# parsakhaz/multimodal-image-similarity-search

Hardware: AMD Instinct MI355X
Metric: images/s CLIP-B/32 encode @ bs256; Mvec/s cosine top-10 over 10M x 512 (higher is better)
Workload: dtype bf16

## Files before the change

### multimodal-image-similarity-search_amd/csrc/attention_common.h

```cpp
#pragma once
#include "common.h"
#include "gemm_fp8.h"

#define ATT_VSTRIDE 144

__device__ __forceinline__ float att_max_over_lane_groups(float v) {
    uint32_t u = __float_as_uint(v);
    auto r32 = __builtin_amdgcn_permlane32_swap(u, u, false, false);
    v = mm_max2(__uint_as_float(r32[0]), __uint_as_float(r32[1]));
    u = __float_as_uint(v);
    auto r16 = __builtin_amdgcn_permlane16_swap(u, u, false, false);
    return mm_max2(__uint_as_float(r16[0]), __uint_as_float(r16[1]));
}

struct AttKV { u32x4 k, v; };
__device__ __forceinline__ AttKV att_load_kv_piece(const uint16_t* base, int ld, int dmodel, int row, int c, int T) {
    AttKV t = {u32x4{0u, 0u, 0u, 0u}, u32x4{0u, 0u, 0u, 0u}};
    if (row < T) {
        t.k = *reinterpret_cast<const u32x4*>(base + (size_t)row * ld + dmodel + c * 8);
        t.v = *reinterpret_cast<const u32x4*>(base + (size_t)row * ld + 2 * dmodel + c * 8);
    }
    return t;
}
__device__ __forceinline__ void att_store_kv_piece(char* sK, char* sV, int row, int c, const u32x4 kv, const u32x4 vv) {
    *reinterpret_cast<u32x4*>(sK + row * 128 + ((c ^ (row & 7)) << 4)) = kv;
    *reinterpret_cast<u32x4*>(sV + row * ATT_VSTRIDE + (c << 4)) = vv;
}
template <int ROWS, int NTHR>
__device__ __forceinline__ void att_stage_kv(const uint16_t* base, int ld, int dmodel, int T, int tid, char* sK) {
    for (int idx = tid; idx < ROWS * 8; idx += NTHR) {
        const int row = idx >> 3, c = idx & 7;
        const AttKV t = att_load_kv_piece(base, ld, dmodel, row, c, T);
        att_store_kv_piece(sK, sK + ROWS * 128, row, c, t.k, t.v);
    }
}

__device__ __forceinline__ bf16x8 att_load_q(const uint16_t* base, int ld, int q, int T, int s, int fg) {
    u32x4 raw = {0u, 0u, 0u, 0u};
    if (q < T) raw = *reinterpret_cast<const u32x4*>(base + (size_t)q * ld + s * 32 + fg * 8);
    return __builtin_bit_cast(bf16x8, raw);
}

__device__ __forceinline__ void att_pv_block(const char* vks, const bf16x8& pf, f32x4 (&oacc)[4]) {
#pragma unroll
    for (int dt = 0; dt < 4; ++dt) {
        const char* a0 = vks + dt * 32;
        const bf16x4 v0 = __builtin_amdgcn_ds_read_tr16_b64_v4bf16(
            (__attribute__((address_space(3))) bf16x4*)(a0));
        const bf16x4 v1 = __builtin_amdgcn_ds_read_tr16_b64_v4bf16(
            (__attribute__((address_space(3))) bf16x4*)(a0 + 16 * ATT_VSTRIDE));
        bf16x8 vf;
        vf[0] = v0[0]; vf[1] = v0[1]; vf[2] = v0[2]; vf[3] = v0[3];
        vf[4] = v1[0]; vf[5] = v1[1]; vf[6] = v1[2]; vf[7] = v1[3];
        oacc[dt] = __builtin_amdgcn_mfma_f32_16x16x32_bf16(vf, pf, oacc[dt], 0, 0, 0);
    }
}

#define ATT_C_EXP (0.125f * 1.4426950408889634f)
#define ATT_THR_RAW (8.0f / ATT_C_EXP)

template <bool PAIR, class ScoreTile>
__device__ __forceinline__ void att_key_pair_step(ScoreTile&& score_tile, int ks, const char* vks, const bf16x8& ones, float& m,
                                                  f32x4& lacc, f32x4 (&oacc)[4]) {
    const float c_exp = ATT_C_EXP, thr_raw = ATT_THR_RAW;
    f32x4 p0 = score_tile(2 * ks), p1;
    if constexpr (PAIR) p1 = score_tile(2 * ks + 1);
    else p1 = f32x4{-INFINITY, -INFINITY, -INFINITY, -INFINITY};
    if constexpr (PAIR) mm_mfma_settle("+v"(p0), "+v"(p1));
    else mm_mfma_settle("+v"(p0));
    float lm = mm_max3(p0[0], p0[1], p0[2]);
    if constexpr (PAIR) lm = mm_max3(mm_max3(lm, p0[3], p1[0]), p1[1], mm_max2(p1[2], p1[3]));
    else lm = mm_max2(lm, p0[3]);
    lm = att_max_over_lane_groups(lm);
    if (__any(lm > m + thr_raw)) {
        const float mn = (lm > m + thr_raw) ? lm : m;
        const float alpha = __builtin_amdgcn_exp2f((m - mn) * c_exp);
        m = mn;
#pragma unroll
        for (int dt = 0; dt < 4; ++dt)
#pragma unroll
            for (int r = 0; r < 4; ++r) oacc[dt][r] *= alpha;
#pragma unroll
        for (int r = 0; r < 4; ++r) lacc[r] *= alpha;
    }
    const float mc = m * c_exp;
#pragma unroll
    for (int r = 0; r < 4; ++r) p0[r] = __builtin_amdgcn_exp2f(__builtin_fmaf(p0[r], c_exp, -mc));
#pragma unroll
    for (int r = 0; r < 4; ++r) p1[r] = __builtin_amdgcn_exp2f(__builtin_fmaf(p1[r], c_exp, -mc));
    u32x4 praw;
    praw[0] = pack_bf16x2(p0[0], p0[1]);
    praw[1] = pack_bf16x2(p0[2], p0[3]);
    praw[2] = pack_bf16x2(p1[0], p1[1]);
    praw[3] = pack_bf16x2(p1[2], p1[3]);
    const bf16x8 pf = __builtin_bit_cast(bf16x8, praw);
    lacc = __builtin_amdgcn_mfma_f32_16x16x32_bf16(ones, pf, lacc, 0, 0, 0);
    att_pv_block(vks, pf, oacc);
}

__device__ __forceinline__ void att_store_bf16_row(const f32x4 (&oacc)[4], float inv, uint16_t* orow) {
#pragma unroll
    for (int dt = 0; dt < 4; ++dt) {
        u32x2 pk;
        pk[0] = pack_bf16x2(oacc[dt][0] * inv, oacc[dt][1] * inv);
        pk[1] = pack_bf16x2(oacc[dt][2] * inv, oacc[dt][3] * inv);
        *reinterpret_cast<u32x2*>(orow + dt * 16) = pk;
    }
}

__device__ __forceinline__ void att_store_mx_row(const f32x4 (&oacc)[4], float inv, bool valid, uint8_t* o8row, uint8_t* srow,
                                                 int h, int fg) {
#pragma unroll
    for (int blk = 0; blk < 2; ++blk) {
        float o[2][4];
        float amax = 0.f;
#pragma unroll
        for (int i = 0; i < 2; ++i)
#pragma unroll
            for (int r = 0; r < 4; ++r) {
                o[i][r] = oacc[2 * blk + i][r] * inv;
                amax = fmaxf(amax, fabsf(o[i][r]));
            }
        amax = att_max_over_lane_groups(amax);
        int e8;
        float sinv;
        mx_scale_of(amax, e8, sinv);
        if (valid) {
#pragma unroll
            for (int i = 0; i < 2; ++i)
                *reinterpret_cast<uint32_t*>(o8row + (2 * blk + i) * 16) = pack_fp8x4(o[i][0] * sinv, o[i][1] * sinv, o[i][2] * sinv, o[i][3] * sinv);
            if (fg == 0) srow[mx_scale_offset(2 * h + blk)] = (uint8_t)e8;
        }
    }
}
```

### multimodal-image-similarity-search_amd/csrc/attention_kernels.h

```cpp
#pragma once
#include "attention_common.h"
#include "attention_stream.h"


template <int NKP, bool CAUSAL, bool MXOUT = false>
__device__ __forceinline__ void attention_onepass_tile(const char* sK, const char* sV, const bf16x8 (&qf)[2], int q, int T,
                                                       int fr, int fg, uint16_t* orow, uint8_t* o8row = nullptr, uint8_t* srow = nullptr,
                                                       int h = 0, int only_q = -1) {
    f32x4 sacc[2 * NKP];
    float mx = -INFINITY;
#pragma unroll
    for (int kt = 0; kt < 2 * NKP; ++kt) {
        f32x4 a = {0.f, 0.f, 0.f, 0.f};
        const int krow = kt * 16 + fr;
#pragma unroll
        for (int s = 0; s < 2; ++s) {
            const int chunk = 4 * s + fg;
            const bf16x8 kf = *reinterpret_cast<const bf16x8*>(sK + krow * 128 + ((chunk ^ (krow & 7)) << 4));
            a = __builtin_amdgcn_mfma_f32_16x16x32_bf16(kf, qf[s], a, 0, 0, 0);
        }
#pragma unroll
        for (int r = 0; r < 4; ++r) {
            const int key = kt * 16 + 4 * fg + r;
            const bool ok = (key < T) && (!CAUSAL || key <= q);
            a[r] = ok ? a[r] * 0.125f : -INFINITY;
            mx = fmaxf(mx, a[r]);
        }
        sacc[kt] = a;
    }
    mx = fmaxf(mx, __shfl_xor(mx, 16));
    mx = fmaxf(mx, __shfl_xor(mx, 32));
    float l = 0.f;
#pragma unroll
    for (int kt = 0; kt < 2 * NKP; ++kt)
#pragma unroll
        for (int r = 0; r < 4; ++r) {
            const float pexp = __expf(sacc[kt][r] - mx);
            sacc[kt][r] = pexp;
            l += pexp;
        }
    l += __shfl_xor(l, 16);
    l += __shfl_xor(l, 32);

    f32x4 oacc[4];
#pragma unroll
    for (int dt = 0; dt < 4; ++dt) oacc[dt] = f32x4{0.f, 0.f, 0.f, 0.f};
    const int tq = fr >> 2, tp = fr & 3;
#pragma unroll
    for (int ks = 0; ks < NKP; ++ks) {
        u32x4 praw;
        praw[0] = pack_bf16x2(sacc[2 * ks][0], sacc[2 * ks][1]);
        praw[1] = pack_bf16x2(sacc[2 * ks][2], sacc[2 * ks][3]);
        praw[2] = pack_bf16x2(sacc[2 * ks + 1][0], sacc[2 * ks + 1][1]);
        praw[3] = pack_bf16x2(sacc[2 * ks + 1][2], sacc[2 * ks + 1][3]);
        const bf16x8 pf = __builtin_bit_cast(bf16x8, praw);
#pragma unroll
        for (int dt = 0; dt < 4; ++dt) {
            const char* a0 = sV + (32 * ks + 4 * fg + tq) * ATT_VSTRIDE + (dt * 16 + 4 * tp) * 2;
            const bf16x4 v0 = __builtin_amdgcn_ds_read_tr16_b64_v4bf16(
                (__attribute__((address_space(3))) bf16x4*)(a0));
            const bf16x4 v1 = __builtin_amdgcn_ds_read_tr16_b64_v4bf16(
                (__attribute__((address_space(3))) bf16x4*)(a0 + 16 * ATT_VSTRIDE));
            bf16x8 vf;
            vf[0] = v0[0]; vf[1] = v0[1]; vf[2] = v0[2]; vf[3] = v0[3];
            vf[4] = v1[0]; vf[5] = v1[1]; vf[6] = v1[2]; vf[7] = v1[3];
            oacc[dt] = __builtin_amdgcn_mfma_f32_16x16x32_bf16(vf, pf, oacc[dt], 0, 0, 0);
        }
    }
    const float inv = 1.0f / l;
    if constexpr (MXOUT) {
#pragma unroll
        for (int blk = 0; blk < 2; ++blk) {
            float o[2][4];
            float amax = 0.f;
#pragma unroll
            for (int i = 0; i < 2; ++i)
#pragma unroll
                for (int r = 0; r < 4; ++r) {
                    o[i][r] = oacc[2 * blk + i][r] * inv;
                    amax = fmaxf(amax, fabsf(o[i][r]));
                }
            amax = att_max_over_lane_groups(amax);
            int e8;
            float sinv;
            mx_scale_of(amax, e8, sinv);
            if (q < T) {
#pragma unroll
                for (int i = 0; i < 2; ++i)
                    *reinterpret_cast<uint32_t*>(o8row + (2 * blk + i) * 16) = pack_fp8x4(o[i][0] * sinv, o[i][1] * sinv, o[i][2] * sinv, o[i][3] * sinv);
                if (fg == 0) srow[mx_scale_offset(2 * h + blk)] = (uint8_t)e8;
            }
        }
    } else if (q < T && (only_q < 0 || q == only_q)) {
        att_store_bf16_row(oacc, inv, orow);
    }
}

template <int NKP, bool CAUSAL, bool MXOUT = false>
__global__ __launch_bounds__(256) void attention_kernel(const uint16_t* __restrict__ qkv, uint16_t* __restrict__ ctx, int T, int H,
                                                        uint8_t* __restrict__ ctx8 = nullptr, uint8_t* __restrict__ ctxs = nullptr, int ld_s = 0) {
    static_assert(NKP <= 4, "sequences over 128 keys: attention_long_kernel");
    extern __shared__ __attribute__((aligned(16))) char smem[];
    constexpr int TP = NKP * 32;
    char* sK = smem;
    char* sV = smem + TP * 128;
    const int tid = threadIdx.x, lane = tid & 63, wave = tid >> 6;
    const int b = blockIdx.x / H, h = blockIdx.x - b * H;
    const int dmodel = H * 64, ld = 3 * dmodel;
    const uint16_t* base = qkv + (size_t)b * T * ld + h * 64;

    constexpr int NW = 4;
    const int fr = lane & 15, fg = lane >> 4;
    const int qt_first = wave + NW * blockIdx.y;
    bf16x8 qf_first[2];
#pragma unroll
    for (int s = 0; s < 2; ++s) qf_first[s] = att_load_q(base, ld, qt_first * 16 + fr, T, s, fg);
    att_stage_kv<TP, NW * 64>(base, ld, dmodel, T, tid, sK);
    __syncthreads();

    const int nqt = (T + 15) >> 4;
    for (int qt = qt_first; qt < nqt; qt += NW * gridDim.y) {
        const int q = qt * 16 + fr;
        bf16x8 qf[2];
        if (qt == qt_first) {
            qf[0] = qf_first[0];
            qf[1] = qf_first[1];
        } else {
#pragma unroll
            for (int s = 0; s < 2; ++s) qf[s] = att_load_q(base, ld, q, T, s, fg);
        }
        if constexpr (MXOUT) {
            const size_t row = (size_t)b * T + (q < T ? q : 0);
            attention_onepass_tile<NKP, CAUSAL, true>(sK, sV, qf, q, T, fr, fg, nullptr, ctx8 + row * dmodel + h * 64 + 4 * fg, ctxs + row * ld_s, h);
        } else {
            attention_onepass_tile<NKP, CAUSAL>(sK, sV, qf, q, T, fr, fg, ctx + ((size_t)b * T + q) * dmodel + h * 64 + 4 * fg);
        }
    }
}

template <int NKP, bool CAUSAL, bool MXOUT>
__global__ __launch_bounds__(512) void attention_long_kernel(const uint16_t* __restrict__ qkv, uint16_t* __restrict__ ctx, int T,
                                                             int H, uint8_t* __restrict__ ctx8, uint8_t* __restrict__ ctxs, int ld_s) {
    static_assert(NKP > 4 && NKP <= 9, "129..288 keys");
    extern __shared__ __attribute__((aligned(16))) char smem[];
    constexpr int TP = NKP * 32;
    constexpr int NW = 8;
    char* sK = smem;
    char* sV = smem + TP * 128;
    const int tid = threadIdx.x, lane = tid & 63, wave = tid >> 6;
    const int dmodel = H * 64, ld = 3 * dmodel;
    const int fr = lane & 15, fg = lane >> 4;
    const int nqt = (T + 15) >> 4;
    const char* kbase0 = sK + fr * 128 + ((fg ^ (fr & 7)) << 4);
    const char* kbase1 = sK + fr * 128 + (((4 + fg) ^ (fr & 7)) << 4);
    const int tq = fr >> 2, tp = fr & 3;
    const char* vbase = sV + (4 * fg + tq) * ATT_VSTRIDE + 8 * tp;
    u32x4 ones_raw = {0x3F803F80u, 0x3F803F80u, 0x3F803F80u, 0x3F803F80u};
    asm volatile("" : "+v"(ones_raw));
    const bf16x8 ones = __builtin_bit_cast(bf16x8, ones_raw);

    const int b = blockIdx.x / H, h = blockIdx.x - b * H;
    const uint16_t* base = qkv + (size_t)b * T * ld + h * 64;
    att_stage_kv<TP, NW * 64>(base, ld, dmodel, T, tid, sK);
    __syncthreads();
    for (int qt = wave + NW * blockIdx.y; qt < nqt; qt += NW * gridDim.y) {
        const int q = qt * 16 + fr;
        bf16x8 qf[2];
#pragma unroll
        for (int s = 0; s < 2; ++s) qf[s] = att_load_q(base, ld, q, T, s, fg);
        const int kt_end = CAUSAL ? (qt + 1 < nqt ? qt + 1 : nqt) : nqt;
        const int kt_clean = CAUSAL ? (qt < (T >> 4) ? qt : (T >> 4)) : (T >> 4);
        auto score_tile = [&](int kt) -> f32x4 {
            f32x4 a = {0.f, 0.f, 0.f, 0.f};
            const bf16x8 kf0 = *reinterpret_cast<const bf16x8*>(kbase0 + kt * 2048);
            const bf16x8 kf1 = *reinterpret_cast<const bf16x8*>(kbase1 + kt * 2048);
            a = __builtin_amdgcn_mfma_f32_16x16x32_bf16(kf0, qf[0], a, 0, 0, 0);
            a = __builtin_amdgcn_mfma_f32_16x16x32_bf16(kf1, qf[1], a, 0, 0, 0);
            if (kt >= kt_clean) {
#pragma unroll
                for (int r = 0; r < 4; ++r) {
                    const int key = kt * 16 + 4 * fg + r;
                    const bool ok = (key < T) && (!CAUSAL || key <= q);
                    a[r] = ok ? a[r] : -INFINITY;
                }
            }
            return a;
        };
        float m = -INFINITY;
        f32x4 lacc = {0.f, 0.f, 0.f, 0.f};
        f32x4 oacc[4];
#pragma unroll
        for (int dt = 0; dt < 4; ++dt) oacc[dt] = f32x4{0.f, 0.f, 0.f, 0.f};
        const int npairs = kt_end >> 1;
#pragma unroll 1
        for (int ks = 0; ks < npairs; ++ks) att_key_pair_step<true>(score_tile, ks, vbase + ks * (32 * ATT_VSTRIDE), ones, m, lacc, oacc);
        if (kt_end & 1) att_key_pair_step<false>(score_tile, npairs, vbase + npairs * (32 * ATT_VSTRIDE), ones, m, lacc, oacc);
        const float inv = 1.0f / lacc[0];
        if constexpr (MXOUT) {
            const size_t row = (size_t)b * T + (q < T ? q : 0);
            att_store_mx_row(oacc, inv, q < T, ctx8 + row * dmodel + h * 64 + 4 * fg, ctxs + row * ld_s, h, fg);
        } else if (q < T) {
            att_store_bf16_row(oacc, inv, ctx + ((size_t)b * T + q) * dmodel + h * 64 + 4 * fg);
        }
    }
}

template <int NKP, bool CAUSAL, int HPB, bool MXOUT = false, bool POOLED = false>
__global__ __launch_bounds__(256) void attention_heads_kernel(const uint16_t* __restrict__ qkv, uint16_t* __restrict__ ctx,
                                                              int T, int H, uint8_t* __restrict__ ctx8 = nullptr,
                                                              uint8_t* __restrict__ ctxs = nullptr, int ld_s = 0,
                                                              const int32_t* __restrict__ pool_row = nullptr) {
    static_assert(!(POOLED && MXOUT), "the pooled-query form writes bf16");
    extern __shared__ __attribute__((aligned(16))) char smem[];
    constexpr int TP = NKP * 32;
    constexpr int IMG = TP * (128 + ATT_VSTRIDE);
    const int tid = threadIdx.x, lane = tid & 63, wave = tid >> 6;
    const int fr = lane & 15, fg = lane >> 4;
    const int groups = H / HPB;
    const int b = blockIdx.x / groups, h0 = (blockIdx.x - b * groups) * HPB;
    const int dmodel = H * 64, ld = 3 * dmodel;
    const uint16_t* item = qkv + (size_t)b * T * ld;
    const int nqt = (T + 15) >> 4;

    constexpr int NIT = TP * 8 / 256;
    u32x4 kr[NIT], vr[NIT];
    auto load_head = [&](int h) {
        const uint16_t* base = item + h * 64;
#pragma unroll
        for (int i = 0; i < NIT; ++i) {
            const int idx = tid + i * 256, row = idx >> 3, c = idx & 7;
            kr[i] = u32x4{0u, 0u, 0u, 0u};
            vr[i] = u32x4{0u, 0u, 0u, 0u};
            if (row < T) {
                kr[i] = *reinterpret_cast<const u32x4*>(base + (size_t)row * ld + dmodel + c * 8);
                vr[i] = *reinterpret_cast<const u32x4*>(base + (size_t)row * ld + 2 * dmodel + c * 8);
            }
        }
    };
    auto store_head = [&](int buf) {
        char* sK = smem + buf * IMG;
        char* sV = sK + TP * 128;
#pragma unroll
        for (int i = 0; i < NIT; ++i) {
            const int idx = tid + i * 256, row = idx >> 3, c = idx & 7;
            *reinterpret_cast<u32x4*>(sK + row * 128 + ((c ^ (row & 7)) << 4)) = kr[i];
            *reinterpret_cast<u32x4*>(sV + row * ATT_VSTRIDE + (c << 4)) = vr[i];
        }
    };
    auto load_q = [&](int h, int qt, bf16x8 (&qf)[2]) {
        const int q = qt * 16 + fr;
#pragma unroll
        for (int s = 0; s < 2; ++s) {
            u32x4 raw = {0u, 0u, 0u, 0u};
            if (q < T) raw = *reinterpret_cast<const u32x4*>(item + h * 64 + (size_t)q * ld + s * 32 + fg * 8);
            qf[s] = __builtin_bit_cast(bf16x8, raw);
        }
    };

    bf16x8 qf[2], qn[2];
    int pq = 0, pqt = wave;
    if constexpr (POOLED) {
        pq = __builtin_amdgcn_readfirstlane(pool_row[b]) - b * T;
        pq = pq < 0 ? 0 : (pq >= T ? T - 1 : pq);
        pqt = pq >> 4;
    }
    const bool my_tile = !POOLED || wave == (pqt & 3);
    if constexpr (POOLED) { if (my_tile) load_q(h0, pqt, qf); }
    else load_q(h0, wave, qf);
    load_head(h0);
    store_head(0);
    __syncthreads();
#pragma unroll 1
    for (int hh = 0; hh < HPB; ++hh) {
        const int h = h0 + hh, cur = hh & 1;
        if (hh + 1 < HPB) {
            if constexpr (POOLED) { if (my_tile) load_q(h + 1, pqt, qn); }
            else load_q(h + 1, wave, qn);
            load_head(h + 1);
        }
        const char* sK = smem + cur * IMG;
        const char* sV = sK + TP * 128;
        if constexpr (POOLED) {
            if (my_tile)
                attention_onepass_tile<NKP, CAUSAL>(sK, sV, qf, pqt * 16 + fr, T, fr, fg, ctx + (size_t)b * dmodel + h * 64 + 4 * fg,
                                                    nullptr, nullptr, 0, pq);
        } else
        for (int qt = wave; qt < nqt; qt += 4) {
            const int q = qt * 16 + fr;
            if (qt != wave) load_q(h, qt, qf);
            if constexpr (MXOUT) {
                const size_t row = (size_t)b * T + (q < T ? q : 0);
                attention_onepass_tile<NKP, CAUSAL, true>(sK, sV, qf, q, T, fr, fg, nullptr, ctx8 + row * dmodel + h * 64 + 4 * fg, ctxs + row * ld_s, h);
            } else
            attention_onepass_tile<NKP, CAUSAL>(sK, sV, qf, q, T, fr, fg, ctx + ((size_t)b * T + q) * dmodel + h * 64 + 4 * fg);
        }
        if (hh + 1 < HPB) {
            store_head(cur ^ 1);
            qf[0] = qn[0];
            qf[1] = qn[1];
        }
        __syncthreads();
    }
}

#include "attention_tiled.h"

template <bool MAY_CAUSAL, class F>
static int attention_with_causal(bool causal, F&& f) {
    if constexpr (MAY_CAUSAL)
        if (causal) return f(std::true_type{});
    return f(std::false_type{});
}
template <int LO, int HI, bool MAY_CAUSAL, class F>
static int attention_with_nkp(int T, bool causal, F&& f) {
    if constexpr (LO < HI)
        if ((T + 31) / 32 > LO) return attention_with_nkp<LO + 1, HI, MAY_CAUSAL>(T, causal, f);
    return attention_with_causal<MAY_CAUSAL>(causal, [&](auto causal_tag) -> int { return f(std::integral_constant<int, LO>{}, causal_tag); });
}
template <class F>
static int attention_with_hpb(int hpb, F&& f) {
    switch (hpb) {
        case 2: return f(std::integral_constant<int, 2>{});
        case 3: return f(std::integral_constant<int, 3>{});
        case 4: return f(std::integral_constant<int, 4>{});
        default: return f(std::integral_constant<int, 6>{});
    }
}

static int attention_query_splits(int items, int T, int waves) {
    const int rounds = ((T + 15) / 16 + waves - 1) / waves;
    const int qs = 256 / items;
    return qs < 1 ? 1 : (qs > rounds ? rounds : qs);
}

static int attention_pick_hpb(int B, int H) {
    int hpb = mmiss_option("att_hpb", 0);
    if (hpb == 0) {
        hpb = 1;
        for (int c : {4, 6, 3, 2})
            if (H % c == 0 && (int64_t)B * (H / c) >= 512) { hpb = c; break; }
    }
    return ((hpb == 2 || hpb == 3 || hpb == 4 || hpb == 6) && H % hpb == 0) ? hpb : 1;
}

template <bool MXOUT>
static int launch_attention_short(hipStream_t st, const void* qkv, void* ctx, uint8_t* ctx8, uint8_t* ctxs, int ld_s, int B, int T,
                                  int H, bool causal) {
    const int hpb = attention_pick_hpb(B, H);
    return attention_with_nkp<1, 4, !MXOUT>(T, causal, [&](auto nkp_tag, auto causal_tag) -> int {
        constexpr int NKP = decltype(nkp_tag)::value;
        constexpr bool CAUSAL = decltype(causal_tag)::value;
        constexpr int lds = NKP * 32 * (128 + ATT_VSTRIDE);
        if (hpb > 1)
            return attention_with_hpb(hpb, [&](auto hpb_tag) -> int {
                constexpr int HPB = decltype(hpb_tag)::value;
                MM_TRY(mmiss_ensure_dyn_lds(reinterpret_cast<const void*>(&attention_heads_kernel<NKP, CAUSAL, HPB, MXOUT>), 2 * lds));
                hipLaunchKernelGGL((attention_heads_kernel<NKP, CAUSAL, HPB, MXOUT>), dim3(B * (H / HPB)), dim3(256), 2 * lds, st,
                                   (const uint16_t*)qkv, (uint16_t*)ctx, T, H, ctx8, ctxs, ld_s);
                MM_HIP(hipGetLastError());
                return MMISS_OK;
            });
        MM_TRY(mmiss_ensure_dyn_lds(reinterpret_cast<const void*>(&attention_kernel<NKP, CAUSAL, MXOUT>), lds));
        hipLaunchKernelGGL((attention_kernel<NKP, CAUSAL, MXOUT>), dim3(B * H, attention_query_splits(B * H, T, 4)), dim3(256), lds, st,
                           (const uint16_t*)qkv, (uint16_t*)ctx, T, H, ctx8, ctxs, ld_s);
        MM_HIP(hipGetLastError());
        return MMISS_OK;
    });
}

template <bool MXOUT>
static int launch_attention_long(hipStream_t st, const void* qkv, void* ctx, uint8_t* ctx8, uint8_t* ctxs, int ld_s, int B, int T, int H,
                                 bool causal) {
    if (!causal)
        if (attention_stream_ok(B, T, H, false) && mmiss_option("attention_stream", 1))
            return launch_attention_stream<MXOUT>(st, qkv, ctx, ctx8, ctxs, ld_s, B, H);
    return attention_with_nkp<5, 9, !MXOUT>(T, causal, [&](auto nkp_tag, auto causal_tag) -> int {
        constexpr int NKP = decltype(nkp_tag)::value;
        constexpr bool CAUSAL = decltype(causal_tag)::value;
        constexpr int lds = NKP * 32 * (128 + ATT_VSTRIDE);
        MM_TRY(mmiss_ensure_dyn_lds(reinterpret_cast<const void*>(&attention_long_kernel<NKP, CAUSAL, MXOUT>), lds));
        hipLaunchKernelGGL((attention_long_kernel<NKP, CAUSAL, MXOUT>), dim3(B * H, attention_query_splits(B * H, T, 8)), dim3(512), lds,
                           st, (const uint16_t*)qkv, (uint16_t*)ctx, T, H, ctx8, ctxs, ld_s);
        MM_HIP(hipGetLastError());
        return MMISS_OK;
    });
}

static bool attention_mx_ok(int T, int H) { return T > 0 && T <= MMISS_MAX_TOKENS && H > 0; }
static int launch_attention_mx(hipStream_t st, const void* qkv, uint8_t* ctx8, uint8_t* ctxs, int ld_s, int B, int T, int H) {
    if (B <= 0) return MMISS_OK;
    if (!attention_mx_ok(T, H) || !ctx8 || !ctxs || ld_s < mx_scale_row_bytes(H * 64))
        MM_FAIL(MMISS_ERR_UNSUPPORTED, "attention (MXFP8 output): T=%d (1..%d), H=%d", T, MMISS_MAX_TOKENS, H);
    MM_PROF("attention_mx", st, 4.0 * B * H * (double)T * T * 64, (double)B * T * H * 64 * (2 * 3 + 1));
    if (T <= 128) return launch_attention_short<true>(st, qkv, nullptr, ctx8, ctxs, ld_s, B, T, H, false);
    if (T > 288) return launch_attention_tiled<false, true>(st, qkv, nullptr, ctx8, ctxs, ld_s, B, T, H);
    return launch_attention_long<true>(st, qkv, nullptr, ctx8, ctxs, ld_s, B, T, H, false);
}

static bool attention_pooled_ok(int B, int T, int H) {
    return B > 0 && T > 0 && T <= 128 && H > 0 && attention_pick_hpb(B, H) > 1;
}
static int launch_attention_pooled(hipStream_t st, const void* qkv, void* ctxc, const int32_t* pool_row, int B, int T, int H,
                                   bool causal) {
    if (!attention_pooled_ok(B, T, H) || !pool_row) MM_FAIL(MMISS_ERR_UNSUPPORTED, "attention (pooled query): B=%d T=%d H=%d", B, T, H);
    MM_PROF("attention", st, 4.0 * B * H * (double)T * 64, ((double)B * T * H * 64 * 2 + (double)B * H * 64 * 2) * 2);
    const int hpb = attention_pick_hpb(B, H);
    return attention_with_nkp<1, 4, true>(T, causal, [&](auto nkp_tag, auto causal_tag) -> int {
        return attention_with_hpb(hpb, [&](auto hpb_tag) -> int {
            constexpr int NKP = decltype(nkp_tag)::value, HPB = decltype(hpb_tag)::value;
            constexpr bool CAUSAL = decltype(causal_tag)::value;
            constexpr int lds = 2 * NKP * 32 * (128 + ATT_VSTRIDE);
            MM_TRY(mmiss_ensure_dyn_lds(reinterpret_cast<const void*>(&attention_heads_kernel<NKP, CAUSAL, HPB, false, true>), lds));
            hipLaunchKernelGGL((attention_heads_kernel<NKP, CAUSAL, HPB, false, true>), dim3(B * (H / HPB)), dim3(256), lds, st,
                               (const uint16_t*)qkv, (uint16_t*)ctxc, T, H, (uint8_t*)nullptr, (uint8_t*)nullptr, 0, pool_row);
            MM_HIP(hipGetLastError());
            return MMISS_OK;
        });
    });
}

static int launch_attention(hipStream_t st, const void* qkv, void* ctx, int B, int T, int H, bool causal) {
    if (B <= 0) return MMISS_OK;
    if (T <= 0 || T > MMISS_MAX_TOKENS || H <= 0)
        MM_FAIL(MMISS_ERR_UNSUPPORTED, "attention: T=%d (1..%d), H=%d", T, MMISS_MAX_TOKENS, H);
    MM_PROF("attention", st, 4.0 * B * H * (double)T * T * 64, (double)B * T * H * 64 * 2 * 4);
    if (T <= 128) return launch_attention_short<false>(st, qkv, ctx, nullptr, nullptr, 0, B, T, H, causal);
    if (T > 288)
        return attention_with_causal<true>(causal, [&](auto causal_tag) -> int {
            return launch_attention_tiled<decltype(causal_tag)::value, false>(st, qkv, ctx, nullptr, nullptr, 0, B, T, H);
        });
    return launch_attention_long<false>(st, qkv, ctx, nullptr, nullptr, 0, B, T, H, causal);
}
```

Before: 93750.

## Use buffer resource loads/stores and permlane-packed 128-bit stores in attention

Result: no change. 94310, median of 6 (+0.6%).

```diff
diff --git a/multimodal-image-similarity-search_amd/csrc/attention_common.h b/multimodal-image-similarity-search_amd/csrc/attention_common.h
--- a/multimodal-image-similarity-search_amd/csrc/attention_common.h
+++ b/multimodal-image-similarity-search_amd/csrc/attention_common.h
@@ -108,6 +108,20 @@
     }
 }
 
+__device__ __forceinline__ void att_store_bf16_row_buf16(const f32x4 (&oacc)[4], float inv, __amdgpu_buffer_rsrc_t srd, int voff16) {
+#pragma unroll
+    for (int j = 0; j < 2; ++j) {
+        u32x2 a, b;
+        a[0] = pack_bf16x2(oacc[2 * j][0] * inv, oacc[2 * j][1] * inv);
+        a[1] = pack_bf16x2(oacc[2 * j][2] * inv, oacc[2 * j][3] * inv);
+        b[0] = pack_bf16x2(oacc[2 * j + 1][0] * inv, oacc[2 * j + 1][1] * inv);
+        b[1] = pack_bf16x2(oacc[2 * j + 1][2] * inv, oacc[2 * j + 1][3] * inv);
+        const auto r0 = __builtin_amdgcn_permlane16_swap(a[0], b[0], false, false);
+        const auto r1 = __builtin_amdgcn_permlane16_swap(a[1], b[1], false, false);
+        __builtin_amdgcn_raw_buffer_store_b128(u32x4{r0[0], r1[0], r0[1], r1[1]}, srd, voff16 + j * 64, 0, 0);
+    }
+}
+
 __device__ __forceinline__ void att_store_mx_row(const f32x4 (&oacc)[4], float inv, bool valid, uint8_t* o8row, uint8_t* srow,
                                                  int h, int fg) {
 #pragma unroll
diff --git a/multimodal-image-similarity-search_amd/csrc/attention_kernels.h b/multimodal-image-similarity-search_amd/csrc/attention_kernels.h
--- a/multimodal-image-similarity-search_amd/csrc/attention_kernels.h
+++ b/multimodal-image-similarity-search_amd/csrc/attention_kernels.h
@@ -3,10 +3,10 @@
 #include "attention_stream.h"
 
 
-template <int NKP, bool CAUSAL, bool MXOUT = false>
+template <int NKP, bool CAUSAL, bool MXOUT = false, class RowStore = std::nullptr_t>
 __device__ __forceinline__ void attention_onepass_tile(const char* sK, const char* sV, const bf16x8 (&qf)[2], int q, int T,
                                                        int fr, int fg, uint16_t* orow, uint8_t* o8row = nullptr, uint8_t* srow = nullptr,
-                                                       int h = 0, int only_q = -1) {
+                                                       int h = 0, int only_q = -1, RowStore row_store = nullptr) {
     f32x4 sacc[2 * NKP];
     float mx = -INFINITY;
 #pragma unroll
@@ -91,6 +91,8 @@
                 if (fg == 0) srow[mx_scale_offset(2 * h + blk)] = (uint8_t)e8;
             }
         }
+    } else if constexpr (!std::is_same<RowStore, std::nullptr_t>::value) {
+        row_store(oacc, inv);
     } else if (q < T && (only_q < 0 || q == only_q)) {
         att_store_bf16_row(oacc, inv, orow);
     }
@@ -219,22 +221,19 @@
     const int groups = H / HPB;
     const int b = blockIdx.x / groups, h0 = (blockIdx.x - b * groups) * HPB;
     const int dmodel = H * 64, ld = 3 * dmodel;
-    const uint16_t* item = qkv + (size_t)b * T * ld;
     const int nqt = (T + 15) >> 4;
+    const __amdgpu_buffer_rsrc_t srd = __builtin_amdgcn_make_buffer_rsrc(const_cast<uint16_t*>(qkv + (size_t)b * T * ld), 0, T * ld * 2, 0x00020000);
+    const __amdgpu_buffer_rsrc_t osrd = __builtin_amdgcn_make_buffer_rsrc(
+        (MXOUT || POOLED) ? nullptr : ctx + (size_t)b * T * dmodel, 0, T * dmodel * 2, 0x00020000);
 
     constexpr int NIT = TP * 8 / 256;
     u32x4 kr[NIT], vr[NIT];
     auto load_head = [&](int h) {
-        const uint16_t* base = item + h * 64;
 #pragma unroll
         for (int i = 0; i < NIT; ++i) {
             const int idx = tid + i * 256, row = idx >> 3, c = idx & 7;
-            kr[i] = u32x4{0u, 0u, 0u, 0u};
-            vr[i] = u32x4{0u, 0u, 0u, 0u};
-            if (row < T) {
-                kr[i] = *reinterpret_cast<const u32x4*>(base + (size_t)row * ld + dmodel + c * 8);
-                vr[i] = *reinterpret_cast<const u32x4*>(base + (size_t)row * ld + 2 * dmodel + c * 8);
-            }
+            kr[i] = __builtin_amdgcn_raw_buffer_load_b128(srd, row * ld * 2 + c * 16, (dmodel + h * 64) * 2, 0);
+            vr[i] = __builtin_amdgcn_raw_buffer_load_b128(srd, row * ld * 2 + c * 16, (2 * dmodel + h * 64) * 2, 0);
         }
     };
     auto store_head = [&](int buf) {
@@ -251,13 +250,12 @@
         const int q = qt * 16 + fr;
 #pragma unroll
         for (int s = 0; s < 2; ++s) {
-            u32x4 raw = {0u, 0u, 0u, 0u};
-            if (q < T) raw = *reinterpret_cast<const u32x4*>(item + h * 64 + (size_t)q * ld + s * 32 + fg * 8);
+            const u32x4 raw = __builtin_amdgcn_raw_buffer_load_b128(srd, q * ld * 2 + fg * 16 + s * 64, h * 128, 0);
             qf[s] = __builtin_bit_cast(bf16x8, raw);
         }
     };
 
-    bf16x8 qf[2], qn[2];
+    bf16x8 qn[2];
     int pq = 0, pqt = wave;
     if constexpr (POOLED) {
         pq = __builtin_amdgcn_readfirstlane(pool_row[b]) - b * T;
@@ -265,40 +263,44 @@
         pqt = pq >> 4;
     }
     const bool my_tile = !POOLED || wave == (pqt & 3);
-    if constexpr (POOLED) { if (my_tile) load_q(h0, pqt, qf); }
-    else load_q(h0, wave, qf);
-    load_head(h0);
+    auto fetch = [&](int h) {
+        if constexpr (POOLED) { if (my_tile) load_q(h, pqt, qn); }
+        else load_q(h, wave, qn);
+        load_head(h);
+    };
+    fetch(h0);
     store_head(0);
     __syncthreads();
-#pragma unroll 1
+#pragma unroll
     for (int hh = 0; hh < HPB; ++hh) {
         const int h = h0 + hh, cur = hh & 1;
-        if (hh + 1 < HPB) {
-            if constexpr (POOLED) { if (my_tile) load_q(h + 1, pqt, qn); }
-            else load_q(h + 1, wave, qn);
-            load_head(h + 1);
-        }
+        const bf16x8 qf[2] = {qn[0], qn[1]};
+        bf16x8 qf2[2];
+        if constexpr (NKP > 2 && !POOLED) { if (wave + 4 < nqt) load_q(h, wave + 4, qf2); }
+        if (hh + 1 < HPB) fetch(h + 1);
+        __builtin_amdgcn_sched_barrier(0);
         const char* sK = smem + cur * IMG;
         const char* sV = sK + TP * 128;
         if constexpr (POOLED) {
             if (my_tile)
                 attention_onepass_tile<NKP, CAUSAL>(sK, sV, qf, pqt * 16 + fr, T, fr, fg, ctx + (size_t)b * dmodel + h * 64 + 4 * fg,
                                                     nullptr, nullptr, 0, pq);
-        } else
-        for (int qt = wave; qt < nqt; qt += 4) {
-            const int q = qt * 16 + fr;
-            if (qt != wave) load_q(h, qt, qf);
-            if constexpr (MXOUT) {
-                const size_t row = (size_t)b * T + (q < T ? q : 0);
-                attention_onepass_tile<NKP, CAUSAL, true>(sK, sV, qf, q, T, fr, fg, nullptr, ctx8 + row * dmodel + h * 64 + 4 * fg, ctxs + row * ld_s, h);
-            } else
-            attention_onepass_tile<NKP, CAUSAL>(sK, sV, qf, q, T, fr, fg, ctx + ((size_t)b * T + q) * dmodel + h * 64 + 4 * fg);
-        }
-        if (hh + 1 < HPB) {
-            store_head(cur ^ 1);
-            qf[0] = qn[0];
-            qf[1] = qn[1];
-        }
+        } else {
+            auto tile = [&](int qt, const bf16x8 (&qq)[2]) {
+                const int q = qt * 16 + fr;
+                if constexpr (MXOUT) {
+                    const size_t row = (size_t)b * T + (q < T ? q : 0);
+                    attention_onepass_tile<NKP, CAUSAL, true>(sK, sV, qq, q, T, fr, fg, nullptr, ctx8 + row * dmodel + h * 64 + 4 * fg, ctxs + row * ld_s, h);
+                } else {
+                    const int voff16 = (q * dmodel + h * 64 + 4 * fg) * 2 + ((fg & 1) ? 24 : 0);
+                    attention_onepass_tile<NKP, CAUSAL>(sK, sV, qq, q, T, fr, fg, nullptr, nullptr, nullptr, 0, -1,
+                                                        [&](const f32x4 (&oacc)[4], float inv) { att_store_bf16_row_buf16(oacc, inv, osrd, voff16); });
+                }
+            };
+            tile(wave, qf);
+            if constexpr (NKP > 2) { if (wave + 4 < nqt) tile(wave + 4, qf2); }
+        }
+        if (hh + 1 < HPB) store_head(cur ^ 1);
         __syncthreads();
     }
 }
```
